# Asd-g/AviSynth-JincResize

Hardware: AMD Instinct MI355X
Metric: Mpix/s per GPU (1080p→4K tap=3 Y8); % HBM-read roofline (higher is better)
Workload: dtype f32

## Files before the change

### avisynth-jincresize_amd/csrc/kernel_periodic.hip

```cpp
#include "device_common.hpp"
#include "knobs.h"
#include <utility>

#pragma clang fp contract(off)

namespace jinc {
namespace {

#include "kernel_periodic_common.inc"

constexpr int kTileCols = 64;

template <int FS, int RG = (FS <= 7 ? 8 : 9)>
struct PeriodicCfg {
    static constexpr int kRowGroups = RG;
    static constexpr int kTileRows = FS * kRowGroups;
    static constexpr int kLdsCols = kTileCols + FS;
    static constexpr int kLdsPitch = kLdsCols + 1;
    static constexpr int kLdsRows = kTileRows + FS;
};

template <typename T, int FS, int RG>
__global__ __launch_bounds__(256) void ewa_periodic_kernel(const PeriodicArgs a, const PlaneIO io) {
    using Cfg = PeriodicCfg<FS, RG>;
// ... 898 lines not shown
        "v_pk_mul_f32 %3, %7, %13 op_sel_hi:[0,1]\n\t"
        "v_pk_add_f32 %0, %0, %2\n\tv_pk_add_f32 %1, %1, %3\n\t"
        "v_pk_mul_f32 %2, %7, %14 op_sel_hi:[0,1]\n\t"
        "v_pk_mul_f32 %3, %7, %14 op_sel:[1,0] op_sel_hi:[1,1]\n\t"
        "v_pk_add_f32 %0, %0, %2\n\tv_pk_add_f32 %1, %1, %3"
        : "+v"(acc_a), "+v"(acc_b), "=&v"(ta), "=&v"(tb)
        : "v"(w0), "v"(w1), "v"(w2), "v"(w3), "s"(c0), "s"(c1), "s"(c2), "s"(c3), "s"(c4), "s"(c5), "s"(c6));
}

__device__ __forceinline__ void quad2_row6_inner(f32x2& acc_a, f32x2& acc_b, f32x2 w0, f32x2 w1, f32x2 w2, f32x2 c1, f32x2 c2, f32x2 c3, f32x2 c4) {
    f32x2 ta, tb;
#define JINC_LO(T, W, C) "v_pk_mul_f32 " T ", " W ", " C " op_sel_hi:[0,1]\n\t"
#define JINC_HI(T, W, C) "v_pk_mul_f32 " T ", " W ", " C " op_sel:[1,0] op_sel_hi:[1,1]\n\t"
#define JINC_ADD2 "v_pk_add_f32 %0, %0, %2\n\tv_pk_add_f32 %1, %1, %3\n\t"
    asm(JINC_HI("%2", "%4", "%7") JINC_LO("%3", "%5", "%7") JINC_ADD2
        JINC_LO("%2", "%5", "%8") JINC_HI("%3", "%5", "%8") JINC_ADD2
        JINC_HI("%2", "%5", "%9") JINC_LO("%3", "%6", "%9") JINC_ADD2
        JINC_LO("%2", "%6", "%10") JINC_HI("%3", "%6", "%10")
        "v_pk_add_f32 %0, %0, %2\n\tv_pk_add_f32 %1, %1, %3"
        : "+v"(acc_a), "+v"(acc_b), "=&v"(ta), "=&v"(tb)
        : "v"(w0), "v"(w1), "v"(w2), "s"(c1), "s"(c2), "s"(c3), "s"(c4));
#undef JINC_LO
#undef JINC_HI
#undef JINC_ADD2
}

#define JINC_Q7_EVEN(W, C)                          \
    "v_pk_mul_f32 %2, " W ", " C " op_sel_hi:[0,1]\n\tv_pk_mul_f32 %3, " W ", " C " op_sel:[1,0] op_sel_hi:[1,1]\n\t" \
    "v_pk_add_f32 %0, %0, %2\n\tv_pk_add_f32 %1, %1, %3\n\t"
#define JINC_Q7_ODD(W, WN, C)              \
    "v_pk_mul_f32 %2, " W ", " C " op_sel:[1,0] op_sel_hi:[1,1]\n\tv_pk_mul_f32 %3, " WN ", " C " op_sel_hi:[0,1]\n\t" \
    "v_pk_add_f32 %0, %0, %2\n\tv_pk_add_f32 %1, %1, %3\n\t"
template <int FORM>
__device__ __forceinline__ void quad2_row7_span(f32x2& acc_a, f32x2& acc_b, f32x2 w0, f32x2 w1, f32x2 w2, f32x2 w3, f32x2 c0, f32x2 c1, f32x2 c2, f32x2 c3,
                                                f32x2 c4, f32x2 c5, f32x2 c6) {
    static_assert(FORM >= 0 && FORM <= 3, "span forms of the seven-tap row");
    f32x2 ta, tb;
    if constexpr (FORM == 0) {
        quad2_row7(acc_a, acc_b, w0, w1, w2, w3, c0, c1, c2, c3, c4, c5, c6);
    } else if constexpr (FORM == 1) {
        asm(JINC_Q7_ODD("%4", "%5", "%8") JINC_Q7_EVEN("%5", "%9") JINC_Q7_ODD("%5", "%6", "%10") JINC_Q7_EVEN("%6", "%11")
            JINC_Q7_ODD("%6", "%7", "%12") JINC_Q7_EVEN("%7", "%13") ""
            : "+v"(acc_a), "+v"(acc_b), "=&v"(ta), "=&v"(tb)
            : "v"(w0), "v"(w1), "v"(w2), "v"(w3), "s"(c1), "s"(c2), "s"(c3), "s"(c4), "s"(c5), "s"(c6));
    } else if constexpr (FORM == 2) {
        asm(JINC_Q7_ODD("%4", "%5", "%8") JINC_Q7_EVEN("%5", "%9") JINC_Q7_ODD("%5", "%6", "%10") JINC_Q7_EVEN("%6", "%11")
            JINC_Q7_ODD("%6", "%7", "%12") ""
            : "+v"(acc_a), "+v"(acc_b), "=&v"(ta), "=&v"(tb)
            : "v"(w0), "v"(w1), "v"(w2), "v"(w3), "s"(c1), "s"(c2), "s"(c3), "s"(c4), "s"(c5));
    } else {
        asm(JINC_Q7_EVEN("%4", "%7") JINC_Q7_ODD("%4", "%5", "%8") JINC_Q7_EVEN("%5", "%9") JINC_Q7_ODD("%5", "%6", "%10") ""
            : "+v"(acc_a), "+v"(acc_b), "=&v"(ta), "=&v"(tb)
            : "v"(w1), "v"(w2), "v"(w3), "s"(c2), "s"(c3), "s"(c4), "s"(c5));
    }
}
#undef JINC_Q7_EVEN
#undef JINC_Q7_ODD

template <int SLOT>
__device__ __forceinline__ void quad2_load_row(f32x2 (&w)[24], const float* p) {
    const f32x2* p2 = reinterpret_cast<const f32x2*>(p);
#pragma unroll
    for (int m = 0; m < 4; ++m) w[4 * SLOT + m] = p2[m];
}

template <int U, uint32_t INNER, int NT>
__device__ __forceinline__ void quad2_pixel6(f32x2 (&acc)[4], const f32x2 (&w)[24], const JINC_CONSTANT f32x2* quad) {
    f32x2 ca[16], cb[16];
    quad_fetch(ca, quad, 0);
#define JINC_QUAD2_STEP(LY, CUR, NEXT)                                                                                        \
    if constexpr (LY < 5) quad_fetch(NEXT, quad, LY + 1);                                                                      \
    __builtin_amdgcn_sched_barrier(0);                                                                                         \
    quad_arrived(CUR);                                                                                                         \
    {                                                                                                                          \
        constexpr int S = 4 * ((U + LY) % 6);                                                                                  \
         \
        if constexpr (NT == 7) {                                             \
                                          \
            quad2_row7_span<(INNER >> (2 * (2 * LY))) & 3u>(acc[0], acc[1], w[S], w[S + 1], w[S + 2], w[S + 3], CUR[0], CUR[1], CUR[2], CUR[3], CUR[4], CUR[5], CUR[6]); \
            quad2_row7_span<(INNER >> (2 * (2 * LY + 1))) & 3u>(acc[2], acc[3], w[S], w[S + 1], w[S + 2], w[S + 3], CUR[8], CUR[9], CUR[10], CUR[11], CUR[12], CUR[13], CUR[14]); \
        } else {                                                                                                               \
        if constexpr ((INNER >> (2 * LY)) & 1u)                                                                                \
            quad2_row6_inner(acc[0], acc[1], w[S], w[S + 1], w[S + 2], CUR[1], CUR[2], CUR[3], CUR[4]);                        \
        else                                                                                                                   \
            quad2_row6(acc[0], acc[1], w[S], w[S + 1], w[S + 2], w[S + 3], CUR[0], CUR[1], CUR[2], CUR[3], CUR[4], CUR[5]);    \
        if constexpr ((INNER >> (2 * LY + 1)) & 1u)                                                                            \
            quad2_row6_inner(acc[2], acc[3], w[S], w[S + 1], w[S + 2], CUR[9], CUR[10], CUR[11], CUR[12]);                     \
        else                                                                                                                   \
            quad2_row6(acc[2], acc[3], w[S], w[S + 1], w[S + 2], w[S + 3], CUR[8], CUR[9], CUR[10], CUR[11], CUR[12], CUR[13]); \
        }                                                                                                                      \
    }                                                                                                                          \
    __builtin_amdgcn_sched_barrier(0);
    JINC_QUAD2_STEP(0, ca, cb)
    JINC_QUAD2_STEP(1, cb, ca)
    JINC_QUAD2_STEP(2, ca, cb)
    JINC_QUAD2_STEP(3, cb, ca)
    JINC_QUAD2_STEP(4, ca, cb)
    JINC_QUAD2_STEP(5, cb, ca)
#undef JINC_QUAD2_STEP
}

template <typename T>
__device__ __forceinline__ void store_quad_buf(BufferRsrc rsrc, uint32_t voffset, uint32_t soffset, f32x2 a, f32x2 b, float peak, bool b_ok) {
    if constexpr (std::is_same_v<T, float>) {
        typedef uint32_t u32x2 __attribute__((ext_vector_type(2)));
        __builtin_amdgcn_raw_buffer_store_b64(__builtin_bit_cast(u32x2, a), rsrc, voffset, soffset, 0);
        if (b_ok) __builtin_amdgcn_raw_buffer_store_b64(__builtin_bit_cast(u32x2, b), rsrc, voffset + 8u, soffset, 0);
    } else if constexpr (std::is_same_v<T, uint8_t>) {
        uint32_t w = __builtin_amdgcn_cvt_pk_u8_f32(a.x, 0u, 0u);
        w = __builtin_amdgcn_cvt_pk_u8_f32(a.y, 1u, w);
        w = __builtin_amdgcn_cvt_pk_u8_f32(b.x, 2u, w);
        w = __builtin_amdgcn_cvt_pk_u8_f32(b.y, 3u, w);
        if (b_ok) __builtin_amdgcn_raw_buffer_store_b32(w, rsrc, voffset, soffset, 0);
        else __builtin_amdgcn_raw_buffer_store_b16(static_cast<uint16_t>(w), rsrc, voffset, soffset, 0);
    } else {
        typedef uint32_t u32x2 __attribute__((ext_vector_type(2)));
        const uint32_t lo = round_pair16<T>(a.x, a.y, peak);
        if (b_ok) {
            const u32x2 v = {lo, round_pair16<T>(b.x, b.y, peak)};
            __builtin_amdgcn_raw_buffer_store_b64(v, rsrc, voffset, soffset, 0);
        } else {
            __builtin_amdgcn_raw_buffer_store_b32(lo, rsrc, voffset, soffset, 0);
        }
    }
}

template <typename T>
__device__ __forceinline__ bool edge_tile_of(const PeriodicArgs& a, int tile_x) {
    if constexpr (is_float_sample_v<T>) return false;
    return a.edge.coeffs != nullptr && ((a.edge.n[0] > 0 && tile_x == a.edge.tile_x[0]) || (a.edge.n[1] > 0 && tile_x == a.edge.tile_x[1]));
}

template <typename T, typename Cfg>
__device__ __forceinline__ void stage_edge_column(const PeriodicArgs& a, const PlaneIO& io, float* tile, int tile_x, const char* sbase, int gx0, int gy0,
                                                  int wave, int lane) {
    static_assert(Cfg::kLdsPitch >= Cfg::kLdsCols + 1 && Cfg::kLdsRows <= 64, "a spare word per tile row, one tile row per lane");
    const bool in_front = (a.edge.n[0] > 0 && tile_x == a.edge.tile_x[0] && a.edge.lds_col[0] < 0) || (a.edge.n[1] > 0 && tile_x == a.edge.tile_x[1] && a.edge.lds_col[1] < 0);
    if (in_front && wave == 0 && lane < Cfg::kLdsRows && gx0 > 0) {
        int gy = gy0 + lane;
        gy = gy < a.src_h ? gy : a.src_h - 1;
        tile[lane * Cfg::kLdsPitch - 1] = to_float(reinterpret_cast<const T*>(sbase + static_cast<size_t>(gy) * io.src_pitch)[gx0 - 1]);
    }
}

__device__ __forceinline__ float wave_shl1(float v) {
    return __builtin_bit_cast(float, __builtin_amdgcn_update_dpp(0, __builtin_bit_cast(int, v), 0x130, 0xf, 0xf, false));
}
__device__ __forceinline__ f32x2 wave_shl1(f32x2 v) { return f32x2{wave_shl1(v.x), wave_shl1(v.y)}; }
__device__ __forceinline__ float frame_lo(float v) { return v; }
__device__ __forceinline__ float frame_lo(f32x2 v) { return v.x; }
__device__ __forceinline__ float frame_hi(float v) { return v; }
__device__ __forceinline__ float frame_hi(f32x2 v) { return v.y; }

template <typename T, typename Cfg, int NR, int NC, typename V = float, int ES = 1>
__device__ __forceinline__ void quad2_edge_columns(const PeriodicArgs& a, const PlaneIO& io, const V* tile, int tile_x, int j0, int wave, int lane,
                                                   BufferRsrc drsrc, BufferRsrc drsrc_hi, bool hi_ok) {
    constexpr bool kPair = !std::is_same_v<V, float>;
    constexpr int NCP = (NC + 3) & ~3;
    for (int s = 0; s < 2; ++s) {
        const int n = a.edge.n[s];
        if (n <= 0 || tile_x != a.edge.tile_x[s]) continue;
        const int q = wave & 1, half = (n + 1) >> 1;
        const int k_begin = (wave >> 1) * half, k_end = k_begin + half < n ? k_begin + half : n;
        if (k_begin >= k_end) continue;
        const bool live = lane < Cfg::kTileRows && j0 + lane < a.nj;
        static_assert(Cfg::kLdsRows <= 64, "one tile row per lane");
        const V* wp = tile + ((lane < Cfg::kLdsRows ? lane : 0) * Cfg::kLdsPitch + a.edge.lds_col[s]) * ES;
        V w[NR][NC];
#pragma unroll
        for (int lx = 0; lx < NC; ++lx) w[0][lx] = wp[lx * ES];
#pragma unroll
        for (int ly = 1; ly < NR; ++ly)
#pragma unroll
            for (int lx = 0; lx < NC; ++lx) w[ly][lx] = wave_shl1(w[ly - 1][lx]);
        const uint32_t row_off = static_cast<uint32_t>(a.iy0 + 2 * (j0 + lane) + q) * static_cast<uint32_t>(io.dst_pitch);
        for (int k0 = k_begin; k0 < k_end; k0 += 4) {
            const int nk = k_end - k0 < 4 ? k_end - k0 : 4;
            V r[4];
#pragma unroll
            for (int k = 0; k < 4; ++k) {
                r[k] = V{};
                if (k < nk) {
                    const JINC_CONSTANT float* cs = (const JINC_CONSTANT float*)(a.edge.coeffs) + ((s * PeriodicArgs::EdgeColumns::kMaxPerSide + k0 + k) * 2 + q) * (NR * NCP);
                    V acc = V{};
#pragma unroll
                    for (int ly = 0; ly < NR; ++ly)
#pragma unroll
                        for (int lx = 0; lx < NC; ++lx) acc = acc + w[ly][lx] * cs[ly * NCP + lx];
                    r[k] = acc;
                }
            }
            if (!live) continue;
            const uint32_t voff = row_off + static_cast<uint32_t>(a.edge.x0[s] + k0) * static_cast<uint32_t>(sizeof(T));
            auto store = [&](BufferRsrc d, auto frame) {
                if (nk == 4) {
                    if constexpr (std::is_same_v<T, uint8_t>) {
                        uint32_t v = __builtin_amdgcn_cvt_pk_u8_f32(frame(r[0]), 0u, 0u);
                        v = __builtin_amdgcn_cvt_pk_u8_f32(frame(r[1]), 1u, v);
                        v = __builtin_amdgcn_cvt_pk_u8_f32(frame(r[2]), 2u, v);
                        v = __builtin_amdgcn_cvt_pk_u8_f32(frame(r[3]), 3u, v);
                        __builtin_amdgcn_raw_buffer_store_b32(v, d, voff, 0, 0);
                    } else {
                        typedef uint32_t u32x2 __attribute__((ext_vector_type(2)));
                        const u32x2 v = {round_pair_u16(frame(r[0]), frame(r[1]), io.peak), round_pair_u16(frame(r[2]), frame(r[3]), io.peak)};
                        __builtin_amdgcn_raw_buffer_store_b64(v, d, voff, 0, 0);
                    }
                } else {
#pragma unroll
                    for (int k = 0; k < 3; ++k)
                        if (k < nk) store_sample_buf<T>(d, voff + static_cast<uint32_t>(k * sizeof(T)), 0, frame(r[k]), io.peak);
                }
            };
            store(drsrc, [](V v) { return frame_lo(v); });
            if constexpr (kPair) {
                if (hi_ok) store(drsrc_hi, [](V v) { return frame_hi(v); });
            }
        }
    }
}

template <int H, int StripsPerWave, int MulLead>
struct Quad2ShareTile {
    static constexpr int kTileCols = 128;
    static constexpr int kStripRows = H;
    static constexpr int kStripsPerWave = StripsPerWave;
    static constexpr int kMulLead = MulLead;
    static constexpr int kTileRows = 4 * H * StripsPerWave;
    static constexpr int kLdsCols = kTileCols + 6;
    static constexpr int kLdsSpare = 4;
    static constexpr int kLdsPitch = kLdsCols + kLdsSpare;
    static constexpr int kLdsRows = kTileRows + 5;
    static constexpr int kLdsFloats = 2 * (kLdsSpare + kLdsRows * kLdsPitch);
    static_assert(kLdsPitch % 2 == 0 && kLdsSpare % 2 == 0, "16-byte aligned rows");
    static_assert(8 * H <= 64, "a strip's outputs index one 64-bit mask");
};
template <int RG>
using Quad2ShareCfg = std::conditional_t<RG == 8, Quad2ShareTile<8, 1, 1>, Quad2ShareTile<2, 2, kQuad2ShareClasses>>;

template <int RG>
__host__ __device__ inline bool quad2_share_runs(const PlaneIO& io) { return RG == 8 || io.nframes > 1; }

template <int H>
constexpr uint64_t quad2_share_outs(int r, int c, int k) {
    uint64_t m = 0;
    for (int oy = 0; oy < 2 * H; ++oy)
        for (int ox = 0; ox < 4; ++ox) {
            const int ly = r - (oy >> 1), lx = c - (ox >> 1);
            if (ly < 0 || ly > 5 || lx < 0 || lx > 5) continue;
            if (quad2_share_class(quad2_share_m(ox & 1, lx), quad2_share_m(oy & 1, ly)) == k) m |= uint64_t{1} << (4 * oy + ox);
        }
    return m;
}

template <int H>
constexpr uint64_t quad2_share_opens(int r, int c, int k) {
    const uint64_t outs = r < H ? quad2_share_outs<H>(r, c, k) : 0;
    uint64_t m = 0;
    for (int o = 8 * r; outs != 0 && o < 8 * r + 8; ++o) {
        if (!((outs >> o) & 1u)) continue;
        const int p = o & 1, q = (o >> 2) & 1, lx = c - ((o & 3) >> 1);
        bool first = true;
        for (int l = 0; l < lx; ++l) first = first && quad2_share_class(quad2_share_m(p, l), quad2_share_m(q, 0)) < 0;
        if (first) m |= uint64_t{1} << o;
    }
    return m;
}
constexpr bool quad2_share_row0_opens(int p, int q) {
    for (int l = 0; l < 6; ++l)
        if (quad2_share_class(quad2_share_m(p, l), quad2_share_m(q, 0)) >= 0) return true;
    return false;
}
static_assert(quad2_share_row0_opens(0, 0) && quad2_share_row0_opens(1, 0) && quad2_share_row0_opens(0, 1) && quad2_share_row0_opens(1, 1),
              "no accumulator is zeroed: the first source row of a period row must open all eight of its chains");

template <int H, int R, int C, int K>
__device__ __forceinline__ void quad2_share_mul(f32x2& t, f32x2 s, const f32x2 (&w)[kQuad2ShareClasses / 2]) {
    if constexpr (quad2_share_outs<H>(R, C, K) != 0) {
        if constexpr (K & 1)
            asm("v_pk_mul_f32 %0, %1, %2 op_sel:[0,1] op_sel_hi:[1,1]" : "=v"(t) : "v"(s), "s"(w[K >> 1]));
        else
            asm("v_pk_mul_f32 %0, %1, %2 op_sel_hi:[1,0]" : "=v"(t) : "v"(s), "s"(w[K >> 1]));
    }
}
template <int H, int R, int C, int K>
__device__ __forceinline__ void quad2_share_adds(f32x2 (&acc)[8 * H], f32x2 t) {
    constexpr uint64_t outs = quad2_share_outs<H>(R, C, K), opens = quad2_share_opens<H>(R, C, K);
#pragma unroll
    for (int o = 0; o < 8 * H; ++o)
        if constexpr (outs != 0)
            if (((outs & ~opens) >> o) & 1u) asm("v_pk_add_f32 %0, %0, %1" : "+v"(acc[o]) : "v"(t));
#pragma unroll
    for (int o = 0; o < 8 * H; ++o)
        if constexpr (opens != 0)
            if ((opens >> o) & 1u) acc[o] = t;
}
template <typename Cfg, int R, int C, int K>
__device__ __forceinline__ void quad2_share_step(f32x2 (&acc)[8 * Cfg::kStripRows], f32x2 (&t)[kQuad2ShareClasses], f32x2 s,
                                                 const f32x2 (&w)[kQuad2ShareClasses / 2]) {
    if constexpr (K < kQuad2ShareClasses) quad2_share_mul<Cfg::kStripRows, R, C, K>(t[K], s, w);
    if constexpr (K >= Cfg::kMulLead) quad2_share_adds<Cfg::kStripRows, R, C, K - Cfg::kMulLead>(acc, t[K - Cfg::kMulLead]);
}
template <typename Cfg, int R, int C, int... K>
__device__ __forceinline__ void quad2_share_sample(f32x2 (&acc)[8 * Cfg::kStripRows], f32x2 s, const f32x2 (&w)[kQuad2ShareClasses / 2],
                                                   std::integer_sequence<int, K...>) {
    f32x2 t[kQuad2ShareClasses];
    (quad2_share_step<Cfg, R, C, K>(acc, t, s, w), ...);
}
template <typename Cfg, int R, int... C>
__device__ __forceinline__ void quad2_share_row(f32x2 (&acc)[8 * Cfg::kStripRows], const f32x2* wb, const f32x2 (&w)[kQuad2ShareClasses / 2],
                                                std::integer_sequence<int, C...>) {
    typedef float f32x4 __attribute__((ext_vector_type(4)));
    const f32x4* p4 = reinterpret_cast<const f32x4*>(wb + R * Cfg::kLdsPitch);
    f32x2 row[8];
#pragma unroll
    for (int m = 0; m < 4; ++m) {
        const f32x4 v = p4[m];
        row[2 * m] = f32x2{v.x, v.y};
        row[2 * m + 1] = f32x2{v.z, v.w};
    }
    (quad2_share_sample<Cfg, R, C>(acc, row[C], w, std::make_integer_sequence<int, kQuad2ShareClasses + Cfg::kMulLead>{}), ...);
}
template <typename Cfg, int... R, typename Store>
__device__ __forceinline__ void quad2_share_strip(f32x2 (&acc)[8 * Cfg::kStripRows], const f32x2* wb, const f32x2 (&w)[kQuad2ShareClasses / 2],
                                                  std::integer_sequence<int, R...>, Store&& store) {
    ((quad2_share_row<Cfg, R>(acc, wb, w, std::make_integer_sequence<int, 7>{}), store(std::integral_constant<int, R - 5>{})), ...);
}

template <typename T, int RG>
__device__ __forceinline__ void quad2_share_body(const PeriodicArgs& a, const PlaneIO& io, float* lds) {
    using Cfg = Quad2ShareCfg<RG>;
    f32x2* const tile = reinterpret_cast<f32x2*>(lds) + Cfg::kLdsSpare;
    const int lane = threadIdx.x & 63;
    const int wave = __builtin_amdgcn_readfirstlane(threadIdx.x >> 6);
    int tile_x, tile_y;
    swizzled_tile(tile_x, tile_y);
    const int i0 = tile_x * Cfg::kTileCols;
    const int j0 = tile_y * Cfg::kTileRows;
    const size_t f0 = 2 * static_cast<size_t>(blockIdx.z);
    const bool f1_ok = f0 + 1 < static_cast<size_t>(io.nframes);
    const size_t f1 = f1_ok ? f0 + 1 : f0;
    const bool edge_tile = edge_tile_of<T>(a, tile_x);
    {
        const int gx0 = a.min_sx + i0;
        const int gy0 = a.min_sy + j0;
        const char* sb0 = static_cast<const char*>(io.src) + f0 * io.src_frame_stride;
        const char* sb1 = static_cast<const char*>(io.src) + f1 * io.src_frame_stride;
        constexpr int kRowsPerWave = (Cfg::kLdsRows + 3) / 4;
        constexpr int kDwords = static_cast<int>(sizeof(T));
        constexpr int kLoadLanes = (Cfg::kLdsCols + 3 + 3) / 4;
        static_assert(kLoadLanes <= 64 && 4 * (kLoadLanes - 1) < Cfg::kLdsPitch - 1 && 4 * (kLoadLanes - 2) + 3 < Cfg::kLdsPitch - 1 && Cfg::kLdsSpare > 3,
                      "the last lane's first sample, the other lanes' four and the three samples in front of a row: spare pairs, not the next row's column -1");
        const uint32_t plane_bytes = static_cast<uint32_t>(a.src_h - 1) * static_cast<uint32_t>(io.src_pitch) + static_cast<uint32_t>(a.src_w) * static_cast<uint32_t>(sizeof(T));
        const uint32_t lead0 = static_cast<uint32_t>(reinterpret_cast<uintptr_t>(sb0)) & 3u, lead1 = static_cast<uint32_t>(reinterpret_cast<uintptr_t>(sb1)) & 3u;
        const BufferRsrc rs0 = make_rsrc(const_cast<char*>(sb0) - lead0, (plane_bytes + lead0 + 3u) & ~3u);
        const BufferRsrc rs1 = make_rsrc(const_cast<char*>(sb1) - lead1, (plane_bytes + lead1 + 3u) & ~3u);
        const uint32_t lead[2] = {lead0, lead1};
        const uint32_t voff = static_cast<uint32_t>(lane) * (4u * kDwords);
        uint32_t d[kRowsPerWave][2][kDwords];
        int shift[kRowsPerWave][2];
#pragma unroll
        for (int i = 0; i < kRowsPerWave; ++i) {
            int gy = gy0 + wave + 4 * i;
            gy = gy < a.src_h ? gy : a.src_h - 1;
#pragma unroll
            for (int f = 0; f < 2; ++f) {
                const uint32_t so = lead[f] + static_cast<uint32_t>(gy) * static_cast<uint32_t>(io.src_pitch) + static_cast<uint32_t>(gx0) * static_cast<uint32_t>(sizeof(T));
                shift[i][f] = static_cast<int>((so & 3u) / sizeof(T));
#pragma unroll
                for (int k = 0; k < kDwords; ++k) d[i][f][k] = __builtin_amdgcn_raw_buffer_load_b32(f ? rs1 : rs0, voff + 4u * k, so & ~3u, 0);
            }
        }
        float* const tf = reinterpret_cast<float*>(tile) + 8 * lane;
        auto sample = [&](int i, int f, int b) {
            if constexpr (sizeof(T) == 1) return static_cast<float>((d[i][f][0] >> (8 * b)) & 0xffu);
            else return static_cast<float>((d[i][f][b >> 1] >> (16 * (b & 1))) & 0xffffu);
        };
        if (lane < kLoadLanes) {
#pragma unroll
            for (int i = 0; i < kRowsPerWave; ++i) {
                const int r = wave + 4 * i;
                if (r >= Cfg::kLdsRows) continue;
#pragma unroll
                for (int f = 0; f < 2; ++f) tf[2 * (r * Cfg::kLdsPitch - shift[i][f]) + f] = sample(i, f, 0);
            }
        }
        if (lane < kLoadLanes - 1) {
#pragma unroll
            for (int i = 0; i < kRowsPerWave; ++i) {
                const int r = wave + 4 * i;
                if (r >= Cfg::kLdsRows) continue;
#pragma unroll
                for (int f = 0; f < 2; ++f)
#pragma unroll
                    for (int b = 1; b < 4; ++b) tf[2 * (r * Cfg::kLdsPitch - shift[i][f] + b) + f] = sample(i, f, b);
            }
        }
        if (gx0 + Cfg::kLdsCols > a.src_w) {
            float* const tr = reinterpret_cast<float*>(tile);
#pragma unroll
            for (int i = 0; i < kRowsPerWave; ++i) {
                const int r = wave + 4 * i;
                if (r >= Cfg::kLdsRows) continue;
                int gy = gy0 + r;
                gy = gy < a.src_h ? gy : a.src_h - 1;
                const float v0 = to_float(reinterpret_cast<const T*>(sb0 + static_cast<size_t>(gy) * io.src_pitch)[a.src_w - 1]);
                const float v1 = to_float(reinterpret_cast<const T*>(sb1 + static_cast<size_t>(gy) * io.src_pitch)[a.src_w - 1]);
#pragma unroll
                for (int k = 0; k < (Cfg::kLdsCols + 63) / 64; ++k) {
                    const int c = lane + 64 * k;
                    if (gx0 + c >= a.src_w && c < Cfg::kLdsCols) {
                        tr[2 * (r * Cfg::kLdsPitch + c)] = v0;
                        tr[2 * (r * Cfg::kLdsPitch + c) + 1] = v1;
                    }
                }
            }
        }
        const bool in_front = edge_tile && ((a.edge.n[0] > 0 && tile_x == a.edge.tile_x[0] && a.edge.lds_col[0] < 0) ||
                                            (a.edge.n[1] > 0 && tile_x == a.edge.tile_x[1] && a.edge.lds_col[1] < 0));
        if (in_front && wave == 0 && lane < Cfg::kLdsRows && gx0 > 0) {
            int gy = gy0 + lane;
            gy = gy < a.src_h ? gy : a.src_h - 1;
            float* const tc = reinterpret_cast<float*>(tile + lane * Cfg::kLdsPitch - 1);
            tc[0] = to_float(reinterpret_cast<const T*>(sb0 + static_cast<size_t>(gy) * io.src_pitch)[gx0 - 1]);
            tc[1] = to_float(reinterpret_cast<const T*>(sb1 + static_cast<size_t>(gy) * io.src_pitch)[gx0 - 1]);
        }
    }
    __syncthreads();
    const uint32_t plane_bytes = static_cast<uint32_t>(io.dst_pitch) * a.dst_h;
    const BufferRsrc d0 = make_rsrc(static_cast<char*>(io.dst) + f0 * io.dst_frame_stride, plane_bytes);
    const BufferRsrc d1 = make_rsrc(static_cast<char*>(io.dst) + f1 * io.dst_frame_stride, plane_bytes);
    if (edge_tile) {
        if constexpr (RG == 8) {
            quad2_edge_columns<T, Cfg, 6, 7, f32x2>(a, io, tile, tile_x, j0, wave, lane, d0, d1, f1_ok);
        } else {
            quad2_edge_columns<T, Cfg, 6, 7, float, 2>(a, io, reinterpret_cast<const float*>(tile), tile_x, j0, wave, lane, d0, d0, false);
            if (f1_ok) quad2_edge_columns<T, Cfg, 6, 7, float, 2>(a, io, reinterpret_cast<const float*>(tile) + 1, tile_x, j0, wave, lane, d1, d1, false);
        }
    }
    const int ia = i0 + 2 * lane;
    if (ia >= a.ni) return;
    const bool b_ok = ia + 1 < a.ni;
    f32x2 w[kQuad2ShareClasses / 2];
#pragma unroll
    for (int k = 0; k < kQuad2ShareClasses / 2; ++k) w[k] = f32x2{a.share_w[2 * k], a.share_w[2 * k + 1]};
    const uint32_t xoff = static_cast<uint32_t>(a.ix0 + 2 * ia) * static_cast<uint32_t>(sizeof(T));
    for (int st = 0; st < Cfg::kStripsPerWave; ++st) {
        const int jb = Cfg::kStripRows * (wave * Cfg::kStripsPerWave + st);
        if (j0 + jb >= a.nj) break;
        const f32x2* wb = tile + jb * Cfg::kLdsPitch + 2 * lane;
        f32x2 acc[8 * Cfg::kStripRows];
        quad2_share_strip<Cfg>(acc, wb, w, std::make_integer_sequence<int, Cfg::kStripRows + 5>{}, [&](auto PR) {
            constexpr int pr = decltype(PR)::value;
            if constexpr (pr >= 0) {
                const int j = j0 + jb + pr;
                if (j < a.nj) {
#pragma unroll
                    for (int q = 0; q < 2; ++q) {
                        const uint32_t so = static_cast<uint32_t>(a.iy0 + 2 * j + q) * static_cast<uint32_t>(io.dst_pitch);
                        const f32x2* r = acc + 4 * (2 * pr + q);
                        store_quad_buf<T>(d0, xoff, so, f32x2{r[0].x, r[1].x}, f32x2{r[2].x, r[3].x}, io.peak, b_ok);
                        if (f1_ok) store_quad_buf<T>(d1, xoff, so, f32x2{r[0].y, r[1].y}, f32x2{r[2].y, r[3].y}, io.peak, b_ok);
                    }
                }
            }
        });
    }
}

constexpr uint32_t kQuad2InnerTap3 = PeriodicArgs::kQuadInnerTap3;
template <typename T, uint32_t INNER, int NT>
constexpr bool quad2_share_instance() { return !is_float_sample_v<T> && INNER == kQuad2InnerTap3 && NT == 6; }
template <typename T, int RG, uint32_t INNER, int NT = 6>
__global__ __launch_bounds__(256, (quad2_share_instance<T, INNER, NT>() && RG == 8 ? 4 : 6)) void ewa_periodic_quad2_kernel(const PeriodicArgs a,
                                                                                                                       const PlaneIO io) {
    using Cfg = Quad2Cfg<RG>;
    constexpr int FS = Cfg::FS;
    static_assert(RG % 4 == 0, "the four waves of a workgroup take RG / 4 row groups each");
    constexpr bool kShare = quad2_share_instance<T, INNER, NT>();
    using ShareCfg = Quad2ShareCfg<RG>;
    constexpr int kWords = 2 + Cfg::kLdsRows * Cfg::kLdsPitch;
    if constexpr (kShare && RG == 8) {
        __shared__ __attribute__((aligned(16))) float share_words[ShareCfg::kLdsFloats];
        quad2_share_body<T, RG>(a, io, share_words);
        return;
    }
    __shared__ __attribute__((aligned(16))) float tile_words[kShare && ShareCfg::kLdsFloats > kWords ? ShareCfg::kLdsFloats : kWords];
    if constexpr (kShare) {
        if (quad2_share_runs<RG>(io)) {
            quad2_share_body<T, RG>(a, io, tile_words);
            return;
        }
    }
    float* const tile = tile_words + 2;

    const int lane = threadIdx.x & 63;
    const int wave = __builtin_amdgcn_readfirstlane(threadIdx.x >> 6);
    int tile_x, tile_y;
    swizzled_tile(tile_x, tile_y);
    const int i0 = tile_x * Cfg::kTileCols;
    const int j0 = tile_y * Cfg::kTileRows;
    const size_t frame = blockIdx.z;
    if (skips_frame(a, frame)) return;
    const bool edge_tile = edge_tile_of<T>(a, tile_x);
    {
        const int gx0 = a.min_sx + i0;
        const int gy0 = a.min_sy + j0;
        const char* sbase = static_cast<const char*>(io.src) + frame * io.src_frame_stride;
        constexpr int kRowsPerWave = (Cfg::kLdsRows + 3) / 4;
        constexpr int kColsPerLane = (Cfg::kLdsCols + 63) / 64;
        T staged[kRowsPerWave][kColsPerLane];
        NonFinite<T> nonfinite(a, frame);
#pragma unroll
        for (int i = 0; i < kRowsPerWave; ++i) {
            int gy = gy0 + wave + 4 * i;
            gy = gy < a.src_h ? gy : a.src_h - 1;
            const T* srow = reinterpret_cast<const T*>(sbase + static_cast<size_t>(gy) * io.src_pitch);
#pragma unroll
            for (int k = 0; k < kColsPerLane; ++k) {
                int gx = gx0 + lane + 64 * k;
                gx = gx < a.src_w ? gx : a.src_w - 1;
                staged[i][k] = srow[gx];
            }
        }
#pragma unroll
        for (int i = 0; i < kRowsPerWave; ++i) {
            const int r = wave + 4 * i;
#pragma unroll
            for (int k = 0; k < kColsPerLane; ++k) {
                const int c = lane + 64 * k;
                if (r < Cfg::kLdsRows && c < Cfg::kLdsCols) tile[r * Cfg::kLdsPitch + c] = nonfinite.take(staged[i][k]);
            }
        }
        if constexpr (!is_float_sample_v<T>) {
            if (edge_tile) stage_edge_column<T, Cfg>(a, io, tile, tile_x, sbase, gx0, gy0, wave, lane);
        }
    }
    __syncthreads();
    const BufferRsrc drsrc = make_rsrc(static_cast<char*>(io.dst) + frame * io.dst_frame_stride,
                                       static_cast<uint32_t>(io.dst_pitch) * a.dst_h);
    if constexpr (!is_float_sample_v<T>) {
        if (edge_tile) quad2_edge_columns<T, Cfg, 6, 7>(a, io, tile, tile_x, j0, wave, lane, drsrc, drsrc, false);
    }
    const int ia = i0 + 2 * lane;
    if (ia >= a.ni) return;
    const bool b_ok = ia + 1 < a.ni;

    const JINC_CONSTANT f32x2* quad = (const JINC_CONSTANT f32x2*)(a.quad);
    const float* base = tile + 2 * lane;
    const uint32_t xoff = static_cast<uint32_t>(a.ix0 + 2 * ia) * static_cast<uint32_t>(sizeof(T));

    constexpr int kGroupsPerWave = RG / 4;
    const int g_first = wave * kGroupsPerWave;
    if (j0 + g_first * FS >= a.nj) return;
    f32x2 win[24];
    {
        const float* wb = base + (g_first * FS) * Cfg::kLdsPitch;
        quad2_load_row<0>(win, wb + 0 * Cfg::kLdsPitch);
        quad2_load_row<1>(win, wb + 1 * Cfg::kLdsPitch);
        quad2_load_row<2>(win, wb + 2 * Cfg::kLdsPitch);
        quad2_load_row<3>(win, wb + 3 * Cfg::kLdsPitch);
        quad2_load_row<4>(win, wb + 4 * Cfg::kLdsPitch);
    }
    for (int g = g_first; g < g_first + kGroupsPerWave; ++g) {
        if (j0 + g * FS >= a.nj) break;
        const float* gbase = base + (g * FS) * Cfg::kLdsPitch;
#define JINC_QUAD2_ROW(U)                                                                                          \
    {                                                                                                              \
        quad2_load_row<(U + FS - 1) % FS>(win, gbase + (U + FS - 1) * Cfg::kLdsPitch);                              \
        f32x2 acc[4] = {{0.f, 0.f}, {0.f, 0.f}, {0.f, 0.f}, {0.f, 0.f}};                                            \
        uint32_t zero;                                                                                              \
        asm volatile("s_mov_b32 %0, 0" : "=s"(zero));  \
        quad2_pixel6<U, INNER, NT>(acc, win, quad + zero);                                                          \
        const int j = j0 + g * FS + U;                                                                              \
        if (j < a.nj) {                                                                                             \
            const uint32_t so = static_cast<uint32_t>(a.iy0 + 2 * j) * io.dst_pitch;                                \
            store_quad_buf<T>(drsrc, xoff, so, acc[0], acc[1], io.peak, b_ok);                                      \
            store_quad_buf<T>(drsrc, xoff, so + static_cast<uint32_t>(io.dst_pitch), acc[2], acc[3], io.peak, b_ok); \
        }                                                                                                           \
    }
        JINC_QUAD2_ROW(0) JINC_QUAD2_ROW(1) JINC_QUAD2_ROW(2) JINC_QUAD2_ROW(3) JINC_QUAD2_ROW(4) JINC_QUAD2_ROW(5)
#undef JINC_QUAD2_ROW
    }
}

template <int RG>
struct Quad2x8Cfg {
    static constexpr int FS = 8;
    static constexpr int kTileCols = 128;
    static constexpr int kTileRows = FS * RG;
    static constexpr int kLdsCols = kTileCols + FS;
    static constexpr int kLdsPitch = 138;
    static constexpr int kLdsRows = kTileRows + FS - 1;
};

__device__ __forceinline__ void quad2_row8(f32x2& acc_a, f32x2& acc_b, f32x2 w0, f32x2 w1, f32x2 w2, f32x2 w3, f32x2 w4, f32x2 c0, f32x2 c1,
                                           f32x2 c2, f32x2 c3, f32x2 c4, f32x2 c5, f32x2 c6, f32x2 c7) {
    f32x2 ta, tb;
#define JINC_LO(T, W, C) "v_pk_mul_f32 " T ", " W ", " C " op_sel_hi:[0,1]\n\t"
#define JINC_HI(T, W, C) "v_pk_mul_f32 " T ", " W ", " C " op_sel:[1,0] op_sel_hi:[1,1]\n\t"
#define JINC_ADD2 "v_pk_add_f32 %0, %0, %2\n\tv_pk_add_f32 %1, %1, %3\n\t"
    asm(JINC_LO("%2", "%4", "%9") JINC_HI("%3", "%4", "%9") JINC_ADD2
        JINC_HI("%2", "%4", "%10") JINC_LO("%3", "%5", "%10") JINC_ADD2
        JINC_LO("%2", "%5", "%11") JINC_HI("%3", "%5", "%11") JINC_ADD2
        JINC_HI("%2", "%5", "%12") JINC_LO("%3", "%6", "%12") JINC_ADD2
        JINC_LO("%2", "%6", "%13") JINC_HI("%3", "%6", "%13") JINC_ADD2
        JINC_HI("%2", "%6", "%14") JINC_LO("%3", "%7", "%14") JINC_ADD2
        JINC_LO("%2", "%7", "%15") JINC_HI("%3", "%7", "%15") JINC_ADD2
        JINC_HI("%2", "%7", "%16") JINC_LO("%3", "%8", "%16")
        "v_pk_add_f32 %0, %0, %2\n\tv_pk_add_f32 %1, %1, %3"
        : "+v"(acc_a), "+v"(acc_b), "=&v"(ta), "=&v"(tb)
        : "v"(w0), "v"(w1), "v"(w2), "v"(w3), "v"(w4), "s"(c0), "s"(c1), "s"(c2), "s"(c3), "s"(c4), "s"(c5), "s"(c6), "s"(c7));
#undef JINC_LO
#undef JINC_HI
#undef JINC_ADD2
}

template <int SLOT>
__device__ __forceinline__ void quad2x8_load_row(f32x2 (&w)[40], const float* p) {
    const f32x2* p2 = reinterpret_cast<const f32x2*>(p);
#pragma unroll
    for (int m = 0; m < 5; ++m) w[5 * SLOT + m] = p2[m];
}

template <int U, uint32_t TR8>
__device__ __forceinline__ void quad2_pixel8(f32x2 (&acc)[4], const f32x2 (&w)[40], const JINC_CONSTANT f32x2* quad) {
    f32x2 ca[16], cb[16];
// ... 580 lines not shown
```

Before: 1.164 million.

## Widen quad2 share strips to four source columns per lane with taller tiles

```diff
diff --git a/avisynth-jincresize_amd/csrc/kernel_periodic.hip b/avisynth-jincresize_amd/csrc/kernel_periodic.hip
--- a/avisynth-jincresize_amd/csrc/kernel_periodic.hip
+++ b/avisynth-jincresize_amd/csrc/kernel_periodic.hip
@@ -1074,7 +1074,7 @@
 __device__ __forceinline__ float frame_hi(float v) { return v; }
 __device__ __forceinline__ float frame_hi(f32x2 v) { return v.y; }
 
-template <typename T, typename Cfg, int NR, int NC, typename V = float, int ES = 1>
+template <typename T, typename Cfg, int NR, int NC, typename V = float, int ES = 1, int Rows = Cfg::kTileRows>
 __device__ __forceinline__ void quad2_edge_columns(const PeriodicArgs& a, const PlaneIO& io, const V* tile, int tile_x, int j0, int wave, int lane,
                                                    BufferRsrc drsrc, BufferRsrc drsrc_hi, bool hi_ok) {
     constexpr bool kPair = !std::is_same_v<V, float>;
@@ -1085,9 +1085,10 @@
         const int q = wave & 1, half = (n + 1) >> 1;
         const int k_begin = (wave >> 1) * half, k_end = k_begin + half < n ? k_begin + half : n;
         if (k_begin >= k_end) continue;
-        const bool live = lane < Cfg::kTileRows && j0 + lane < a.nj;
-        static_assert(Cfg::kLdsRows <= 64, "one tile row per lane");
-        const V* wp = tile + ((lane < Cfg::kLdsRows ? lane : 0) * Cfg::kLdsPitch + a.edge.lds_col[s]) * ES;
+        constexpr int kRows = Rows == Cfg::kTileRows ? Cfg::kLdsRows : Rows + NR - 1;
+        const bool live = lane < Rows && j0 + lane < a.nj;
+        static_assert(kRows <= 64 && kRows <= Cfg::kLdsRows, "one tile row per lane");
+        const V* wp = tile + ((lane < kRows ? lane : 0) * Cfg::kLdsPitch + a.edge.lds_col[s]) * ES;
         V w[NR][NC];
 #pragma unroll
         for (int lx = 0; lx < NC; ++lx) w[0][lx] = wp[lx * ES];
@@ -1141,49 +1142,57 @@
     }
 }
 
-template <int H, int StripsPerWave, int MulLead>
+template <int H, int W, int StripsPerWave, int MulLead>
 struct Quad2ShareTile {
     static constexpr int kTileCols = 128;
     static constexpr int kStripRows = H;
+    static constexpr int kStripCols = W;
+    static constexpr int kWinCols = W + 5;
+    static constexpr int kLanesX = kTileCols / W;
+    static constexpr int kLaneStrips = 64 / kLanesX;
     static constexpr int kStripsPerWave = StripsPerWave;
     static constexpr int kMulLead = MulLead;
-    static constexpr int kTileRows = 4 * H * StripsPerWave;
+    static constexpr int kTileRows = 4 * H * StripsPerWave * kLaneStrips;
+    static constexpr int kEdgeRows = kTileRows + 5 <= 64 ? kTileRows : 32;
     static constexpr int kLdsCols = kTileCols + 6;
     static constexpr int kLdsSpare = 4;
     static constexpr int kLdsPitch = kLdsCols + kLdsSpare;
     static constexpr int kLdsRows = kTileRows + 5;
     static constexpr int kLdsFloats = 2 * (kLdsSpare + kLdsRows * kLdsPitch);
     static_assert(kLdsPitch % 2 == 0 && kLdsSpare % 2 == 0, "16-byte aligned rows");
-    static_assert(8 * H <= 64, "a strip's outputs index one 64-bit mask");
+    static_assert(W % 2 == 0 && kLanesX * W == kTileCols && kLanesX * kLaneStrips == 64 && W * (kLanesX - 1) + ((kWinCols + 1) & ~1) <= kLdsPitch,
+                  "16-byte aligned windows, whole waves, the last lane's window loads inside its row");
+    static_assert(4 * W * H <= 128 && kTileRows % kEdgeRows == 0, "a strip's outputs index one 128-bit mask");
 };
+typedef unsigned __int128 Quad2ShareMask;
 template <int RG>
-using Quad2ShareCfg = std::conditional_t<RG == 8, Quad2ShareTile<8, 1, 1>, Quad2ShareTile<2, 2, kQuad2ShareClasses>>;
+using Quad2ShareCfg = std::conditional_t<RG == 8, Quad2ShareTile<8, 4, 1, 1>, Quad2ShareTile<2, 2, 2, kQuad2ShareClasses>>;
 
 template <int RG>
 __host__ __device__ inline bool quad2_share_runs(const PlaneIO& io) { return RG == 8 || io.nframes > 1; }
 
-template <int H>
-constexpr uint64_t quad2_share_outs(int r, int c, int k) {
-    uint64_t m = 0;
+template <int H, int W>
+constexpr Quad2ShareMask quad2_share_outs(int r, int c, int k) {
+    Quad2ShareMask m = 0;
     for (int oy = 0; oy < 2 * H; ++oy)
-        for (int ox = 0; ox < 4; ++ox) {
+        for (int ox = 0; ox < 2 * W; ++ox) {
             const int ly = r - (oy >> 1), lx = c - (ox >> 1);
             if (ly < 0 || ly > 5 || lx < 0 || lx > 5) continue;
-            if (quad2_share_class(quad2_share_m(ox & 1, lx), quad2_share_m(oy & 1, ly)) == k) m |= uint64_t{1} << (4 * oy + ox);
+            if (quad2_share_class(quad2_share_m(ox & 1, lx), quad2_share_m(oy & 1, ly)) == k) m |= Quad2ShareMask{1} << (2 * W * oy + ox);
         }
     return m;
 }
 
-template <int H>
-constexpr uint64_t quad2_share_opens(int r, int c, int k) {
-    const uint64_t outs = r < H ? quad2_share_outs<H>(r, c, k) : 0;
-    uint64_t m = 0;
-    for (int o = 8 * r; outs != 0 && o < 8 * r + 8; ++o) {
+template <int H, int W>
+constexpr Quad2ShareMask quad2_share_opens(int r, int c, int k) {
+    const Quad2ShareMask outs = r < H ? quad2_share_outs<H, W>(r, c, k) : 0;
+    Quad2ShareMask m = 0;
+    for (int o = 4 * W * r; outs != 0 && o < 4 * W * (r + 1); ++o) {
         if (!((outs >> o) & 1u)) continue;
-        const int p = o & 1, q = (o >> 2) & 1, lx = c - ((o & 3) >> 1);
+        const int p = o & 1, q = (o / (2 * W)) & 1, lx = c - ((o % (2 * W)) >> 1);
         bool first = true;
         for (int l = 0; l < lx; ++l) first = first && quad2_share_class(quad2_share_m(p, l), quad2_share_m(q, 0)) < 0;
-        if (first) m |= uint64_t{1} << o;
+        if (first) m |= Quad2ShareMask{1} << o;
     }
     return m;
 }
@@ -1195,47 +1204,49 @@
 static_assert(quad2_share_row0_opens(0, 0) && quad2_share_row0_opens(1, 0) && quad2_share_row0_opens(0, 1) && quad2_share_row0_opens(1, 1),
               "no accumulator is zeroed: the first source row of a period row must open all eight of its chains");
 
-template <int H, int R, int C, int K>
+template <int H, int W, int R, int C, int K>
 __device__ __forceinline__ void quad2_share_mul(f32x2& t, f32x2 s, const f32x2 (&w)[kQuad2ShareClasses / 2]) {
-    if constexpr (quad2_share_outs<H>(R, C, K) != 0) {
+    if constexpr (quad2_share_outs<H, W>(R, C, K) != 0) {
         if constexpr (K & 1)
             asm("v_pk_mul_f32 %0, %1, %2 op_sel:[0,1] op_sel_hi:[1,1]" : "=v"(t) : "v"(s), "s"(w[K >> 1]));
         else
             asm("v_pk_mul_f32 %0, %1, %2 op_sel_hi:[1,0]" : "=v"(t) : "v"(s), "s"(w[K >> 1]));
     }
 }
-template <int H, int R, int C, int K>
-__device__ __forceinline__ void quad2_share_adds(f32x2 (&acc)[8 * H], f32x2 t) {
-    constexpr uint64_t outs = quad2_share_outs<H>(R, C, K), opens = quad2_share_opens<H>(R, C, K);
-#pragma unroll
-    for (int o = 0; o < 8 * H; ++o)
+template <int H, int W, int R, int C, int K>
+__device__ __forceinline__ void quad2_share_adds(f32x2 (&acc)[4 * W * H], f32x2 t) {
+    constexpr Quad2ShareMask outs = quad2_share_outs<H, W>(R, C, K), opens = quad2_share_opens<H, W>(R, C, K);
+    constexpr uint64_t adds[2] = {static_cast<uint64_t>(outs & ~opens), static_cast<uint64_t>((outs & ~opens) >> 64)};
+    constexpr uint64_t first[2] = {static_cast<uint64_t>(opens), static_cast<uint64_t>(opens >> 64)};
+#pragma unroll
+    for (int o = 0; o < 4 * W * H; ++o)
         if constexpr (outs != 0)
-            if (((outs & ~opens) >> o) & 1u) asm("v_pk_add_f32 %0, %0, %1" : "+v"(acc[o]) : "v"(t));
-#pragma unroll
-    for (int o = 0; o < 8 * H; ++o)
+            if ((adds[o >> 6] >> (o & 63)) & 1u) asm("v_pk_add_f32 %0, %0, %1" : "+v"(acc[o]) : "v"(t));
+#pragma unroll
+    for (int o = 0; o < 4 * W * H; ++o)
         if constexpr (opens != 0)
-            if ((opens >> o) & 1u) acc[o] = t;
+            if ((first[o >> 6] >> (o & 63)) & 1u) acc[o] = t;
 }
 template <typename Cfg, int R, int C, int K>
-__device__ __forceinline__ void quad2_share_step(f32x2 (&acc)[8 * Cfg::kStripRows], f32x2 (&t)[kQuad2ShareClasses], f32x2 s,
+__device__ __forceinline__ void quad2_share_step(f32x2 (&acc)[4 * Cfg::kStripCols * Cfg::kStripRows], f32x2 (&t)[kQuad2ShareClasses], f32x2 s,
                                                  const f32x2 (&w)[kQuad2ShareClasses / 2]) {
-    if constexpr (K < kQuad2ShareClasses) quad2_share_mul<Cfg::kStripRows, R, C, K>(t[K], s, w);
-    if constexpr (K >= Cfg::kMulLead) quad2_share_adds<Cfg::kStripRows, R, C, K - Cfg::kMulLead>(acc, t[K - Cfg::kMulLead]);
+    if constexpr (K < kQuad2ShareClasses) quad2_share_mul<Cfg::kStripRows, Cfg::kStripCols, R, C, K>(t[K], s, w);
+    if constexpr (K >= Cfg::kMulLead) quad2_share_adds<Cfg::kStripRows, Cfg::kStripCols, R, C, K - Cfg::kMulLead>(acc, t[K - Cfg::kMulLead]);
 }
 template <typename Cfg, int R, int C, int... K>
-__device__ __forceinline__ void quad2_share_sample(f32x2 (&acc)[8 * Cfg::kStripRows], f32x2 s, const f32x2 (&w)[kQuad2ShareClasses / 2],
+__device__ __forceinline__ void quad2_share_sample(f32x2 (&acc)[4 * Cfg::kStripCols * Cfg::kStripRows], f32x2 s, const f32x2 (&w)[kQuad2ShareClasses / 2],
                                                    std::integer_sequence<int, K...>) {
     f32x2 t[kQuad2ShareClasses];
     (quad2_share_step<Cfg, R, C, K>(acc, t, s, w), ...);
 }
 template <typename Cfg, int R, int... C>
-__device__ __forceinline__ void quad2_share_row(f32x2 (&acc)[8 * Cfg::kStripRows], const f32x2* wb, const f32x2 (&w)[kQuad2ShareClasses / 2],
+__device__ __forceinline__ void quad2_share_row(f32x2 (&acc)[4 * Cfg::kStripCols * Cfg::kStripRows], const f32x2* wb, const f32x2 (&w)[kQuad2ShareClasses / 2],
                                                 std::integer_sequence<int, C...>) {
     typedef float f32x4 __attribute__((ext_vector_type(4)));
     const f32x4* p4 = reinterpret_cast<const f32x4*>(wb + R * Cfg::kLdsPitch);
-    f32x2 row[8];
-#pragma unroll
-    for (int m = 0; m < 4; ++m) {
+    f32x2 row[(Cfg::kWinCols + 1) & ~1];
+#pragma unroll
+    for (int m = 0; m < (Cfg::kWinCols + 1) / 2; ++m) {
         const f32x4 v = p4[m];
         row[2 * m] = f32x2{v.x, v.y};
         row[2 * m + 1] = f32x2{v.z, v.w};
@@ -1243,9 +1254,9 @@
     (quad2_share_sample<Cfg, R, C>(acc, row[C], w, std::make_integer_sequence<int, kQuad2ShareClasses + Cfg::kMulLead>{}), ...);
 }
 template <typename Cfg, int... R, typename Store>
-__device__ __forceinline__ void quad2_share_strip(f32x2 (&acc)[8 * Cfg::kStripRows], const f32x2* wb, const f32x2 (&w)[kQuad2ShareClasses / 2],
+__device__ __forceinline__ void quad2_share_strip(f32x2 (&acc)[4 * Cfg::kStripCols * Cfg::kStripRows], const f32x2* wb, const f32x2 (&w)[kQuad2ShareClasses / 2],
                                                   std::integer_sequence<int, R...>, Store&& store) {
-    ((quad2_share_row<Cfg, R>(acc, wb, w, std::make_integer_sequence<int, 7>{}), store(std::integral_constant<int, R - 5>{})), ...);
+    ((quad2_share_row<Cfg, R>(acc, wb, w, std::make_integer_sequence<int, Cfg::kWinCols>{}), store(std::integral_constant<int, R - 5>{})), ...);
 }
 
 template <typename T, int RG>
@@ -1339,12 +1350,15 @@
         }
         const bool in_front = edge_tile && ((a.edge.n[0] > 0 && tile_x == a.edge.tile_x[0] && a.edge.lds_col[0] < 0) ||
                                             (a.edge.n[1] > 0 && tile_x == a.edge.tile_x[1] && a.edge.lds_col[1] < 0));
-        if (in_front && wave == 0 && lane < Cfg::kLdsRows && gx0 > 0) {
-            int gy = gy0 + lane;
-            gy = gy < a.src_h ? gy : a.src_h - 1;
-            float* const tc = reinterpret_cast<float*>(tile + lane * Cfg::kLdsPitch - 1);
-            tc[0] = to_float(reinterpret_cast<const T*>(sb0 + static_cast<size_t>(gy) * io.src_pitch)[gx0 - 1]);
-            tc[1] = to_float(reinterpret_cast<const T*>(sb1 + static_cast<size_t>(gy) * io.src_pitch)[gx0 - 1]);
+        if (in_front && wave == 0 && gx0 > 0) {
+#pragma unroll
+            for (int r = lane; r < Cfg::kLdsRows; r += 64) {
+                int gy = gy0 + r;
+                gy = gy < a.src_h ? gy : a.src_h - 1;
+                float* const tc = reinterpret_cast<float*>(tile + r * Cfg::kLdsPitch - 1);
+                tc[0] = to_float(reinterpret_cast<const T*>(sb0 + static_cast<size_t>(gy) * io.src_pitch)[gx0 - 1]);
+                tc[1] = to_float(reinterpret_cast<const T*>(sb1 + static_cast<size_t>(gy) * io.src_pitch)[gx0 - 1]);
+            }
         }
     }
     __syncthreads();
@@ -1353,35 +1367,46 @@
     const BufferRsrc d1 = make_rsrc(static_cast<char*>(io.dst) + f1 * io.dst_frame_stride, plane_bytes);
     if (edge_tile) {
         if constexpr (RG == 8) {
-            quad2_edge_columns<T, Cfg, 6, 7, f32x2>(a, io, tile, tile_x, j0, wave, lane, d0, d1, f1_ok);
+            for (int jp = 0; jp < Cfg::kTileRows && j0 + jp < a.nj; jp += Cfg::kEdgeRows)
+                quad2_edge_columns<T, Cfg, 6, 7, f32x2, 1, Cfg::kEdgeRows>(a, io, tile + jp * Cfg::kLdsPitch, tile_x, j0 + jp, wave, lane, d0, d1, f1_ok);
         } else {
             quad2_edge_columns<T, Cfg, 6, 7, float, 2>(a, io, reinterpret_cast<const float*>(tile), tile_x, j0, wave, lane, d0, d0, false);
             if (f1_ok) quad2_edge_columns<T, Cfg, 6, 7, float, 2>(a, io, reinterpret_cast<const float*>(tile) + 1, tile_x, j0, wave, lane, d1, d1, false);
         }
     }
-    const int ia = i0 + 2 * lane;
+    constexpr int W = Cfg::kStripCols;
+    const int lx = lane % Cfg::kLanesX, ls = lane / Cfg::kLanesX;
+    const int ia = i0 + W * lx;
     if (ia >= a.ni) return;
-    const bool b_ok = ia + 1 < a.ni;
+    const int nv = a.ni - ia;
     f32x2 w[kQuad2ShareClasses / 2];
 #pragma unroll
     for (int k = 0; k < kQuad2ShareClasses / 2; ++k) w[k] = f32x2{a.share_w[2 * k], a.share_w[2 * k + 1]};
-    const uint32_t xoff = static_cast<uint32_t>(a.ix0 + 2 * ia) * static_cast<uint32_t>(sizeof(T));
+    const uint32_t xoff = static_cast<uint32_t>(a.ix0 + 2 * ia) * static_cast<uint32_t>(sizeof(T)) +
+                          static_cast<uint32_t>(2 * Cfg::kStripRows * ls) * static_cast<uint32_t>(io.dst_pitch);
     for (int st = 0; st < Cfg::kStripsPerWave; ++st) {
-        const int jb = Cfg::kStripRows * (wave * Cfg::kStripsPerWave + st);
-        if (j0 + jb >= a.nj) break;
-        const f32x2* wb = tile + jb * Cfg::kLdsPitch + 2 * lane;
-        f32x2 acc[8 * Cfg::kStripRows];
+        const int jw = Cfg::kStripRows * Cfg::kLaneStrips * (wave * Cfg::kStripsPerWave + st);
+        const int jb = jw + Cfg::kStripRows * ls;
+        const int rows = a.nj - j0 - jb;
+        if (rows <= 0) break;
+        const f32x2* wb = tile + jb * Cfg::kLdsPitch + W * lx;
+        f32x2 acc[4 * W * Cfg::kStripRows];
         quad2_share_strip<Cfg>(acc, wb, w, std::make_integer_sequence<int, Cfg::kStripRows + 5>{}, [&](auto PR) {
             constexpr int pr = decltype(PR)::value;
             if constexpr (pr >= 0) {
-                const int j = j0 + jb + pr;
-                if (j < a.nj) {
+                if (pr < rows) {
 #pragma unroll
                     for (int q = 0; q < 2; ++q) {
-                        const uint32_t so = static_cast<uint32_t>(a.iy0 + 2 * j + q) * static_cast<uint32_t>(io.dst_pitch);
-                        const f32x2* r = acc + 4 * (2 * pr + q);
-                        store_quad_buf<T>(d0, xoff, so, f32x2{r[0].x, r[1].x}, f32x2{r[2].x, r[3].x}, io.peak, b_ok);
-                        if (f1_ok) store_quad_buf<T>(d1, xoff, so, f32x2{r[0].y, r[1].y}, f32x2{r[2].y, r[3].y}, io.peak, b_ok);
+                        const uint32_t so = static_cast<uint32_t>(a.iy0 + 2 * (j0 + jw + pr) + q) * static_cast<uint32_t>(io.dst_pitch);
+                        const f32x2* r = acc + 2 * W * (2 * pr + q);
+#pragma unroll
+                        for (int h = 0; h < W; h += 2) {
+                            if (h > 0 && nv <= h) break;
+                            const uint32_t xo = xoff + static_cast<uint32_t>(2 * h * sizeof(T));
+                            const bool b_ok = nv > h + 1;
+                            store_quad_buf<T>(d0, xo, so, f32x2{r[2 * h].x, r[2 * h + 1].x}, f32x2{r[2 * h + 2].x, r[2 * h + 3].x}, io.peak, b_ok);
+                            if (f1_ok) store_quad_buf<T>(d1, xo, so, f32x2{r[2 * h].y, r[2 * h + 1].y}, f32x2{r[2 * h + 2].y, r[2 * h + 3].y}, io.peak, b_ok);
+                        }
                     }
                 }
             }
@@ -1393,7 +1418,7 @@
 template <typename T, uint32_t INNER, int NT>
 constexpr bool quad2_share_instance() { return !is_float_sample_v<T> && INNER == kQuad2InnerTap3 && NT == 6; }
 template <typename T, int RG, uint32_t INNER, int NT = 6>
-__global__ __launch_bounds__(256, (quad2_share_instance<T, INNER, NT>() && RG == 8 ? 4 : 6)) void ewa_periodic_quad2_kernel(const PeriodicArgs a,
+__global__ __launch_bounds__(256, (quad2_share_instance<T, INNER, NT>() && RG == 8 ? 2 : 6)) void ewa_periodic_quad2_kernel(const PeriodicArgs a,
                                                                                                                        const PlaneIO io) {
     using Cfg = Quad2Cfg<RG>;
     constexpr int FS = Cfg::FS;
```

Result: faster. 1.179 million, median of 4 (+1.3%).
